# ViTAE-Transformer/MTP

Hardware: AMD Instinct MI355X
Metric: images/sec pretrain step (ViT-L+RVSA, 224^2, bf16) (higher is better)
Workload: dtype bf16; 1 GPU; ViT-L + RVSA backbone fwd+bwd + grad all-reduce + clip + AdamW, 224x224, batch 64 per GPU (BASELINE configs[2]/[3]); global_batch=64, parallelism=dp1, activation_checkpointing=False, heads=sum_i mean(f_i)

## Files before the change

### mtp_amd/csrc/elementwise.hip

```cpp
#include "common.h"

namespace {

template <typename T, bool INVERSE>
__global__ __launch_bounds__(256) void patchify_kernel(float* __restrict__ img, T* __restrict__ cols, int B, int Cin, int H, int W, int P, int Hp, int Wp) {
    const int K4 = Cin * P * P / 4, P4 = P / 4;
    const int64_t total = (int64_t)B * Hp * Wp * K4;
    for (int64_t i = (int64_t)blockIdx.x * 256 + threadIdx.x; i < total; i += (int64_t)gridDim.x * 256) {
        const int k4 = (int)(i % K4);
        const int64_t t = i / K4;
        const int kx4 = k4 % P4, ky = (k4 / P4) % P, c = k4 / (P4 * P);
        const int px = (int)(t % Wp), py = (int)((t / Wp) % Hp), b = (int)(t / ((int64_t)Wp * Hp));
        float* ip = img + (((int64_t)b * Cin + c) * H + py * P + ky) * W + px * P + kx4 * 4;
        T* cp = cols + t * (K4 * 4) + k4 * 4;
        if (INVERSE)
            *reinterpret_cast<float4*>(ip) = load4(cp);
        else
            store4(cp, *reinterpret_cast<const float4*>(ip));
    }
}

template <typename Ts, typename Td>
__global__ __launch_bounds__(256) void cast_kernel(const Ts* __restrict__ s, Td* __restrict__ d, int64_t n) {
    const int64_t n4 = n >> 2;
// ... 46 lines not shown
                }
            }
        }
    } else {
        const int64_t c = c0 + a;
        if (c < C) {
            const Tin* rp = ib + c * S + s0 + g;
#pragma unroll
            for (int v = 0; v < 4; ++v) {
                const int64_t s2 = s0 + g + 4 * v;
                if (s2 + 3 < S && (S & 3) == 0) {
                    const float4 x = load4(rp + 4 * v);
                    tile[a][g + 4 * v] = x.x; tile[a][g + 4 * v + 1] = x.y; tile[a][g + 4 * v + 2] = x.z; tile[a][g + 4 * v + 3] = x.w;
                } else {
                    for (int e = 0; e < 4; ++e)
                        if (s2 + e < S) tile[a][g + 4 * v + e] = Elem<Tin>::load(rp + 4 * v + e);
                }
            }
        }
        __syncthreads();
        const int64_t s = s0 + a;
        if (s < S) {
            Tout* wp = ob + pixel_to_row(s, Wp, L) * C + c0 + g;
#pragma unroll
            for (int v = 0; v < 4; ++v)
                if (c0 + g + 4 * v < C)
                    store4(wp + 4 * v, make_float4(tile[g + 4 * v][a], tile[g + 4 * v + 1][a], tile[g + 4 * v + 2][a], tile[g + 4 * v + 3][a]));
        }
    }
}

template <bool ROWS2COLS>
__global__ __launch_bounds__(256) void transpose8_bf16_kernel(const bf16_t* __restrict__ in, bf16_t* __restrict__ out, int64_t S, int64_t C, int Wp, int L) {
    __shared__ float tile[64][65];
    const int64_t bt = blockIdx.z;
    const int64_t s0 = (int64_t)blockIdx.x * 64, c0 = (int64_t)blockIdx.y * 64;
    const bf16_t* ib = in + bt * S * C;
    bf16_t* ob = out + bt * S * C;
    const int t = threadIdx.x, ra = t >> 3, cg = (t & 7) * 8;
    float x[8];
    if (ROWS2COLS) {
#pragma unroll
        for (int h = 0; h < 2; ++h) {
            const int64_t sp = s0 + ra + 32 * h;
            if (sp < S && c0 + cg < C) {
                load8(ib + pixel_to_row(sp, Wp, L) * C + c0 + cg, x);
#pragma unroll
                for (int e = 0; e < 8; ++e) tile[cg + e][ra + 32 * h] = x[e];
            }
        }
        __syncthreads();
#pragma unroll
        for (int h = 0; h < 2; ++h) {
            const int64_t c = c0 + ra + 32 * h;
            if (c < C && s0 + cg < S) {
#pragma unroll
                for (int e = 0; e < 8; ++e) x[e] = tile[ra + 32 * h][cg + e];
                store8(ob + c * S + s0 + cg, x);
            }
        }
    } else {
#pragma unroll
        for (int h = 0; h < 2; ++h) {
            const int64_t c = c0 + ra + 32 * h;
            if (c < C && s0 + cg < S) {
                load8(ib + c * S + s0 + cg, x);
#pragma unroll
                for (int e = 0; e < 8; ++e) tile[ra + 32 * h][cg + e] = x[e];
            }
        }
        __syncthreads();
#pragma unroll
        for (int h = 0; h < 2; ++h) {
            const int64_t sp = s0 + ra + 32 * h;
            if (sp < S && c0 + cg < C) {
#pragma unroll
                for (int e = 0; e < 8; ++e) x[e] = tile[cg + e][ra + 32 * h];
                store8(ob + pixel_to_row(sp, Wp, L) * C + c0 + cg, x);
            }
        }
    }
}

template <bool ROWS2COLS>
int launch_transpose(const void* in, int in_dt, void* out, int out_dt, int64_t batches, int64_t S, int64_t C, int Wp, int L, hipStream_t s) {
    if (C % 4) return MTP_ERR_ARG;
    dim3 grid((unsigned)((S + 63) / 64), (unsigned)((C + 63) / 64), (unsigned)batches), block(256);
    if (in_dt == MTP_BF16 && out_dt == MTP_BF16 && !(S & 7) && !(C & 7) && !(((uintptr_t)in | (uintptr_t)out) & 15)) {
        transpose8_bf16_kernel<ROWS2COLS><<<grid, block, 0, s>>>((const bf16_t*)in, (bf16_t*)out, S, C, Wp, L);
        return mtp_launch_status();
    }
    MTP_DISPATCH2(in_dt, out_dt, transpose_kernel<TA, TB, ROWS2COLS><<<grid, block, 0, s>>>((const TA*)in, (TB*)out, S, C, Wp, L));
    return mtp_launch_status();
}

template <typename T>
__global__ __launch_bounds__(256) void convt_pack_kernel(const float* __restrict__ w, T* __restrict__ wg, T* __restrict__ wgT, int64_t Cin, int64_t Cout) {
    const int64_t total = Cin * Cout * 4;
    for (int64_t i = (int64_t)blockIdx.x * 256 + threadIdx.x; i < total; i += (int64_t)gridDim.x * 256) {
        const int q = (int)(i & 3);
        const int64_t co = (i >> 2) % Cout, ci = (i >> 2) / Cout;
        const float v = w[i];
        if (wg) Elem<T>::store(wg + (q * Cout + co) * Cin + ci, v);
        if (wgT) Elem<T>::store(wgT + ci * (4 * Cout) + q * Cout + co, v);
    }
}
__global__ __launch_bounds__(256) void convt_unpack_kernel(const float* __restrict__ dwg, float* __restrict__ dw, int64_t Cin, int64_t Cout) {
    const int64_t total = Cin * Cout * 4;
    for (int64_t i = (int64_t)blockIdx.x * 256 + threadIdx.x; i < total; i += (int64_t)gridDim.x * 256) {
        const int q = (int)(i & 3);
        const int64_t co = (i >> 2) % Cout, ci = (i >> 2) / Cout;
        dw[i] = dwg[(q * Cout + co) * Cin + ci];
    }
}

template <typename T>
__global__ __launch_bounds__(256) void convt_pack_tiled_kernel(const float* __restrict__ w, T* __restrict__ wg, T* __restrict__ wgT, int Cin, int Cout) {
    __shared__ float tile[2][64][65];
    const int ci0 = blockIdx.y * 64, co0 = blockIdx.x * 64;
    const int t = threadIdx.x, lane = t & 63, wave = t >> 6, ra = t >> 3, cg = (t & 7) * 8;
    float4 v[16];
#pragma unroll
    for (int k = 0; k < 16; ++k) {
        const int ci = ci0 + wave + 4 * k, co = co0 + lane;
        v[k] = (ci < Cin && co < Cout) ? load4(w + ((int64_t)ci * Cout + co) * 4) : make_float4(0.f, 0.f, 0.f, 0.f);
    }
#pragma unroll
    for (int half = 0; half < 2; ++half) {
        if (half) __syncthreads();
#pragma unroll
        for (int k = 0; k < 16; ++k) {
            tile[0][wave + 4 * k][lane] = half ? v[k].z : v[k].x;
            tile[1][wave + 4 * k][lane] = half ? v[k].w : v[k].y;
        }
        __syncthreads();
        float o[8];
        if (wgT) {
            for (int l = ra; l < 128; l += 32) {
                const int r = l >> 1, qq = l & 1, ci = ci0 + r;
                if (ci < Cin && co0 + cg < Cout) {
#pragma unroll
                    for (int e = 0; e < 8; ++e) o[e] = tile[qq][r][cg + e];
                    store8(wgT + (int64_t)ci * 4 * Cout + (int64_t)(2 * half + qq) * Cout + co0 + cg, o);
                }
            }
        }
        if (wg) {
            for (int l = ra; l < 128; l += 32) {
                const int qq = l >> 6, c = l & 63, co = co0 + c;
                if (co < Cout && ci0 + cg < Cin) {
#pragma unroll
                    for (int e = 0; e < 8; ++e) o[e] = tile[qq][cg + e][c];
                    store8(wg + ((int64_t)(2 * half + qq) * Cout + co) * Cin + ci0 + cg, o);
                }
            }
        }
    }
}
__global__ __launch_bounds__(256) void convt_unpack_tiled_kernel(const float* __restrict__ dwg, float* __restrict__ dw, int Cin, int Cout) {
    __shared__ float tile[2][64][65];
    const int ci0 = blockIdx.y * 64, co0 = blockIdx.x * 64;
    const int t = threadIdx.x, lane = t & 63, wave = t >> 6, rb = t >> 4, c4 = (t & 15) * 4;
    float g[16][4];
#pragma unroll
    for (int half = 0; half < 2; ++half) {
        if (half) __syncthreads();
        for (int l = rb; l < 128; l += 16) {
            const int qq = l >> 6, c = l & 63, co = co0 + c;
            if (co < Cout && ci0 + c4 < Cin) {
                const float4 x = load4(dwg + ((int64_t)(2 * half + qq) * Cout + co) * Cin + ci0 + c4);
                tile[qq][c4 + 0][c] = x.x; tile[qq][c4 + 1][c] = x.y; tile[qq][c4 + 2][c] = x.z; tile[qq][c4 + 3][c] = x.w;
            }
        }
        __syncthreads();
// ... 280 lines not shown
```

### mtp_amd/engine.py

```python
import os

import torch

from . import ops
from .engine_base import EngineBase

F32 = torch.float32


class _Blk:
    __slots__ = ("window", "pre", "wqkv", "wqkvT", "wproj", "wprojT", "w1", "w1T", "w2", "w2T", "wsamp", "bsamp", "bproj", "b2", "wproj_s", "w2_s")


class BackboneEngine(EngineBase):
    def __init__(self, module, act_dtype=torch.bfloat16):
        super().__init__(module, act_dtype)
        self.C = module.embed_dim
        self.depth = len(module.blocks)
        self.heads = module.num_heads
        self.hd = self.C // self.heads
        self.scale = module.qk_scale if module.qk_scale is not None else self.hd ** -0.5
        self.window = [bool(w) for w in module.window_blocks]
        self.out_indices = list(module.out_indices)
        self._blk = None
        self._fpn = None
        self._pe = None
        self._ls = []
        self._zero_rel = {}

    def _fold_sources(self, P):
        with torch.no_grad():
            for pre, b in self._ls:
                g1, g2 = P[pre + "gamma_1"].detach(), P[pre + "gamma_2"].detach()
                torch.mul(P[pre + "attn.proj.weight"].detach(), g1[:, None], out=b.wproj_s)
                torch.mul(P[pre + "mlp.fc2.weight"].detach(), g2[:, None], out=b.w2_s)
                torch.mul(P[pre + "attn.proj.bias"].detach(), g1, out=b.bproj)
                torch.mul(P[pre + "mlp.fc2.bias"].detach(), g2, out=b.b2)

    def _pack_weights(self, P):
        for name, (wg, wgT) in self._fpn.items():
            ops.convt_pack(P[name + ".weight"].detach().contiguous(), wg, wgT)

    def fusable_images(self):
        return None if self._ls else self._wimg

    def _build_weight_images(self, P):
        dev = P["patch_embed.proj.weight"].device
        act, H, C = self.act, self.heads, self.C
        entries = []

        def both(w2d):
            w2d = w2d.detach()
            assert w2d.is_contiguous()
            R, Cc = w2d.shape
            wt = torch.empty(Cc, R, device=dev, dtype=act)
            w = w2d if act == F32 else torch.empty(R, Cc, device=dev, dtype=act)
            entries.append((w2d, None if act == F32 else w, wt, False))
            return w, wt

        ls = getattr(self.m, "init_values", None) is not None
        self._ls = []

        blks = []
        for i in range(self.depth):
            b = _Blk()
            b.window = self.window[i]
            b.pre = pre = "blocks.%d." % i
            b.wqkv, b.wqkvT = both(P[pre + "attn.qkv.weight"])
            b.bproj, b.b2 = P[pre + "attn.proj.bias"].detach(), P[pre + "mlp.fc2.bias"].detach()
            if ls:
                b.wproj_s, b.w2_s = torch.empty_like(P[pre + "attn.proj.weight"]), torch.empty_like(P[pre + "mlp.fc2.weight"])
                b.bproj, b.b2 = torch.empty_like(P[pre + "attn.proj.bias"]), torch.empty_like(P[pre + "mlp.fc2.bias"])
                self._ls.append((pre, b))
                b.wproj, b.wprojT = both(b.wproj_s)
            else:
                b.wproj, b.wprojT = both(P[pre + "attn.proj.weight"])
            b.w1, b.w1T = both(P[pre + "mlp.fc1.weight"])
            b.w2, b.w2T = both(b.w2_s if ls else P[pre + "mlp.fc2.weight"])
            if b.window:
                b.wsamp = torch.empty(5 * H, C, device=dev, dtype=F32)
                b.bsamp = torch.empty(5 * H, device=dev, dtype=F32)
                r0 = 0
                for head, rows in (("sampling_offsets", 2 * H), ("sampling_scales", 2 * H), ("sampling_angles", H)):
                    entries.append((P[pre + "attn.%s.2.weight" % head].detach().view(rows, C), b.wsamp[r0:r0 + rows], None, True))
                    entries.append((P[pre + "attn.%s.2.bias" % head].detach().view(1, rows), b.bsamp[r0:r0 + rows], None, True))
                    r0 += rows
            blks.append(b)
        self._blk = blks
        wpe = P["patch_embed.proj.weight"].detach()
        self._pe = both(wpe.view(wpe.shape[0], -1))
        fpn = {}
        for name in ("fpn1.0", "fpn1.3", "fpn2.0"):
            if name + ".weight" in P:
                Cin, Cout = P[name + ".weight"].shape[:2]
                fpn[name] = (torch.empty(4 * Cout, Cin, device=dev, dtype=act), torch.empty(Cin, 4 * Cout, device=dev, dtype=act))
        self._fpn = fpn
        self._wimg = ops.WeightImages(entries, act)

    wgrad_side_stream = True
    wgrad_max_jobs = 8
    wgrad_keep = 2

    @staticmethod
    def _colsum(dy, out):
        return ops.colsum(dy, out, accumulate=True)

    def _ln_bwd(self, *args, **kw):
        return ops.layernorm_bwd(*args, accumulate=True, defer=self._ln_parts, **kw)

    def _full_rel(self, pre, Hp, Wp):
        h = self.P.get(pre + "attn.full_attn_rel_pos_h")
        if h is not None:
            w = self.P[pre + "attn.full_attn_rel_pos_w"]
            if h.shape[0] < 2 * Hp - 1 or w.shape[0] < 2 * Wp - 1:
                raise ValueError("%sattn.full_attn_rel_pos_h/w have %d / %d rows, a %d x %d token grid needs %d / %d (resize them like "
                                 "init_weights does, or build the model for this input size)" % (pre, h.shape[0], w.shape[0], Hp, Wp, 2 * Hp - 1, 2 * Wp - 1))
            return h[:2 * Hp - 1], w[:2 * Wp - 1]
        key = (Hp, Wp)
        if self._zero_rel.get(key) is None:
            self._zero_rel[key] = (torch.zeros(2 * Hp - 1, self.hd, device=self.dev, dtype=F32),
                                   torch.zeros(2 * Wp - 1, self.hd, device=self.dev, dtype=F32))
        return self._zero_rel[key]

    def _drop_scales(self, B, training):
        rates = [float(self.m.drop_path_rates[i]) for i in range(self.depth)]
        live = [training and r > 0.0 and self.m.blocks[i].training for i, r in enumerate(rates)]
        if not any(live):
            return [(None, None)] * self.depth
        keep = torch.tensor([1.0 - r for r in rates], dtype=F32).to(self.dev, non_blocking=True).view(self.depth, 1, 1)
        s = torch.floor(keep + torch.rand(self.depth, 2, B, device=self.dev, dtype=F32)) / keep
        return [(s[i, 0], s[i, 1]) if live[i] else (None, None) for i in range(self.depth)]

    @property
    def _ride(self):
        return self.act == torch.bfloat16 and not self.m.use_checkpoint

    def _block_fwd(self, i, x, B, Hp, Wp, dps, save):
        P, b, C, T, N = self.P, self._blk[i], self.C, x.shape[0], Hp * Wp
        pre = b.pre
        s = {}
        mean1, rstd1 = self._e(T, dtype=F32), self._e(T, dtype=F32)
        ln1 = ops.layernorm_fwd(x, P[pre + "norm1.weight"], P[pre + "norm1.bias"], self._e(T, C), mean1, rstd1)
        rider = None
        if b.window:
            nh, nw = ops.rvsa_windows(Hp, Wp)
            R = B * nh * nw
            avg, pooled = self._e(R, C, dtype=F32), self._e(R, C, dtype=F32)
            samp = self._e(R, 5 * self.heads, dtype=F32)
            if self._ride:
                rider = ops.sampling_fwd_rider(ln1, b.wsamp, b.bsamp, avg, pooled, samp, B, Hp, Wp)
            else:
                ops.rvsa_sampling_fwd(ln1, b.wsamp, b.bsamp, avg, pooled, samp, B, Hp, Wp)
        qkv = ops.gemm_nt(ln1, b.wqkv, self._e(T, 3 * C), bias=P[pre + "attn.qkv.bias"], rider=rider)
        o = self._e(T, C)
        if b.window:
            lse = self._e(R * self.heads * 49, dtype=F32)
            ops.rvsa_attn_fwd(qkv, samp, o, lse, P[pre + "attn.rel_pos_h"], P[pre + "attn.rel_pos_w"],
                              P[pre + "attn.relative_position_bias_table"], B, Hp, Wp, self.heads, self.scale)
            s.update(avg=avg, pooled=pooled, samp=samp)
        else:
            lse = self._e(B * self.heads * N, dtype=F32)
            rel_h, rel_w = self._full_rel(pre, Hp, Wp)
            ops.full_attn_fwd(qkv, o, lse, rel_h, rel_w, B, Hp, Wp, self.heads, self.scale)
        x1 = ops.gemm_nt(o, b.wproj, self._e(T, C, dtype=F32), epi=ops.EPI_BIAS_RES, bias=b.bproj, res=x,
                         rowscale=dps[0], rows_per_sample=N)
        mean2, rstd2 = self._e(T, dtype=F32), self._e(T, dtype=F32)
        ln2 = ops.layernorm_fwd(x1, P[pre + "norm2.weight"], P[pre + "norm2.bias"], self._e(T, C), mean2, rstd2)
        u = self._e(T, 4 * C)
        h = ops.gemm_nt(ln2, b.w1, self._e(T, 4 * C), epi=ops.EPI_BIAS_GELU_DG, bias=P[pre + "mlp.fc1.bias"], aux=u)
        x2 = ops.gemm_nt(h, b.w2, self._e(T, C, dtype=F32), epi=ops.EPI_BIAS_RES, bias=b.b2, res=x1,
                         rowscale=dps[1], rows_per_sample=N)
        if save:
            s.update(x=x, mean1=mean1, rstd1=rstd1, ln1=ln1, qkv=qkv, o=o, lse=lse, x1=x1, mean2=mean2, rstd2=rstd2, ln2=ln2, u=u, h=h)
        return x2, s

    def _layer_scale_grads(self, pre, lin, gname, G):
        P = self.P
        gw, gb, gam = G[pre + lin + ".weight"], G[pre + lin + ".bias"], P[pre + gname]
        G[pre + gname].add_((gw * P[pre + lin + ".weight"]).sum(1) + gb * P[pre + lin + ".bias"])
        gw.mul_(gam[:, None])
        gb.mul_(gam)

    def _block_bwd(self, i, s, dx2, dx2_act, B, Hp, Wp, dps, G, extra, prev_scale):
        P, b, C, N = self.P, self._blk[i], self.C, Hp * Wp
        pre = b.pre
        T = dx2.shape[0]
        wq = self._wq
        ls = pre + "gamma_1" in G
# ... 66 lines not shown
        else:
            B, Cin, H, W = img.shape
            Hp, Wp = H // ps, W // ps
            N, T = Hp * Wp, B * Hp * Wp
            img = img.contiguous()
            if img.dtype != F32:
                img = img.float()
            cols = ops.patchify(img, self._e(T, Cin * ps * ps), ps)
        pos = P.get("pos_embed")
        if pos is not None:
            assert pos.shape[1] == N, "pos_embed does not match the input size"
            x = ops.gemm_nt(cols, self._pe[0], self._e(T, C, dtype=F32), epi=ops.EPI_BIAS_RES, bias=P["patch_embed.proj.bias"],
                            res=pos.reshape(N, C), res_mod=N)
        else:
            x = ops.gemm_nt(cols, self._pe[0], self._e(T, C, dtype=F32), bias=P["patch_embed.proj.bias"])
        dps = self._drop_scales(B, training)
        ckpt = bool(m.use_checkpoint) and need_grad
        saved, taps = [], {}
        vitdet = bool(getattr(m, "_vitdet", False))
        last = self.depth - 1 if vitdet else max(self.out_indices)
        for i in range(self.depth):
            if i > last:
                break
            xin = x
            x, s = self._block_fwd(i, x, B, Hp, Wp, dps[i], save=need_grad and not ckpt)
            saved.append(s if (need_grad and not ckpt) else ({"x": xin} if need_grad else None))
            if i in self.out_indices:
                taps[i] = x
        final = None
        if vitdet:
            fm, fr = self._e(T, dtype=F32), self._e(T, dtype=F32)
            xn = ops.layernorm_fwd(x, P["norm.weight"], P["norm.bias"], self._e(T, C, dtype=F32), fm, fr)
            final = (x, fm, fr)
            tap_list = [xn, xn, xn, xn]
        else:
            tap_list = [taps[i] for i in self.out_indices]
        if getattr(m, "_taps_only", False):
            feats = [ops.tokens_to_nchw(t, self._e(B, C, Hp, Wp, dtype=fdt), B, Hp, Wp, 0) for t in tap_list]
            fctx = {"taps_only": True}
        else:
            feats, fctx = self._fpn_fwd(tap_list, B, Hp, Wp, fdt, need_grad)
        ctx = None
        if need_grad:
            ctx = dict(saved=saved, dps=dps, fctx=fctx, cols=cols, geom=(B, Cin, H, W, Hp, Wp), ckpt=ckpt, last=last, final=final)
        return feats, ctx

    def _fpn_fwd(self, taps, B, Hp, Wp, fdt, need_grad):
        P, C, T = self.P, self.C, B * Hp * Wp
        m = self.m
        feats, fctx = [], {}
        if m.patch_size == 8:
            t0 = taps[0] if self.act == F32 else ops.cast(taps[0], self._e(T, C))
            z = ops.gemm_nt(t0, self._fpn["fpn1.0"][0], self._e(T, 4 * C), bias=P["fpn1.0.bias"], bias_mod=C)
            feats.append(ops.tokens_to_nchw(z.view(4 * T, C), self._e(B, C, 2 * Hp, 2 * Wp, dtype=fdt), B, Hp, Wp, 1))
            feats.append(ops.tokens_to_nchw(taps[1], self._e(B, C, Hp, Wp, dtype=fdt), B, Hp, Wp, 0))
            H2, W2, H4, W4 = Hp // 2, Wp // 2, Hp // 4, Wp // 4
            p3 = ops.maxpool2_tokens_fwd(taps[2], self._e(B * H2 * W2, C), B, Hp, Wp)
            feats.append(ops.tokens_to_nchw(p3, self._e(B, C, H2, W2, dtype=fdt), B, H2, W2, 0))
            q1 = ops.maxpool2_tokens_fwd(taps[3], self._e(B * H2 * W2, C, dtype=F32), B, Hp, Wp)
            q2 = ops.maxpool2_tokens_fwd(q1, self._e(B * H4 * W4, C), B, H2, W2)
            feats.append(ops.tokens_to_nchw(q2, self._e(B, C, H4, W4, dtype=fdt), B, H4, W4, 0))
            if need_grad:
                fctx = dict(p8=True, t0=t0, tap2=taps[2], tap3=taps[3], q1=q1)
            return feats, fctx
        if m.patch_size != 16:
            raise NotImplementedError("the reference defines the FPN tail for patch_size 16 and 8 only (VIT:640-670)")
        t0 = taps[0] if self.act == F32 else ops.cast(taps[0], self._e(T, C))
        y1 = ops.gemm_nt(t0, self._fpn["fpn1.0"][0], self._e(T, 4 * C), bias=P["fpn1.0.bias"], bias_mod=C)
        mean, rstd = self._e(4 * T, dtype=F32), self._e(4 * T, dtype=F32)
        g1 = ops.layernorm_fwd(y1.view(4 * T, C), P["fpn1.1.ln.weight"], P["fpn1.1.ln.bias"], self._e(4 * T, C), mean, rstd, gelu=True)
        y2 = ops.gemm_nt(g1, self._fpn["fpn1.3"][0], self._e(4 * T, 4 * C), bias=P["fpn1.3.bias"], bias_mod=C)
        feats.append(ops.tokens_to_nchw(y2.view(16 * T, C), self._e(B, C, 4 * Hp, 4 * Wp, dtype=fdt), B, Hp, Wp, 2))
        t1 = taps[1] if self.act == F32 else ops.cast(taps[1], self._e(T, C))
        z = ops.gemm_nt(t1, self._fpn["fpn2.0"][0], self._e(T, 4 * C), bias=P["fpn2.0.bias"], bias_mod=C)
        feats.append(ops.tokens_to_nchw(z.view(4 * T, C), self._e(B, C, 2 * Hp, 2 * Wp, dtype=fdt), B, Hp, Wp, 1))
        feats.append(ops.tokens_to_nchw(taps[2], self._e(B, C, Hp, Wp, dtype=fdt), B, Hp, Wp, 0))
        Ho, Wo = Hp // 2, Wp // 2
        pooled = ops.maxpool2_tokens_fwd(taps[3], self._e(B * Ho * Wo, C), B, Hp, Wp)
        feats.append(ops.tokens_to_nchw(pooled, self._e(B, C, Ho, Wo, dtype=fdt), B, Ho, Wo, 0))
        if need_grad:
            fctx = dict(t0=t0, y1=y1, mean=mean, rstd=rstd, g1=g1, t1=t1, tap3=taps[3])
        return feats, fctx

    def _convt_wgrad(self, dy, x, gw):
        dwg = self._e(dy.shape[1], x.shape[1], dtype=F32)
        self._wq.add(dy, x, dwg, after=lambda: ops.convt_unpack_grad(dwg, gw), norm_of=gw)

    def _fpn_bwd(self, dfeats, fctx, B, Hp, Wp, G):
        P, C, T, act = self.P, self.C, B * Hp * Wp, self.act
        out = [None] * 4

        def as_in(df):
            df = df.contiguous()
            return df if df.dtype in (F32, torch.bfloat16) else df.float()

        if fctx.get("p8"):
            H2, W2, H4, W4 = Hp // 2, Wp // 2, Hp // 4, Wp // 4
            if dfeats[0] is not None:
                dz = ops.nchw_to_tokens(as_in(dfeats[0]), self._e(4 * T, C), B, Hp, Wp, 1)
                self._convt_wgrad(dz.view(T, 4 * C), fctx["t0"], G["fpn1.0.weight"])
                self._colsum(dz, G["fpn1.0.bias"])
                out[0] = ops.gemm_nt(dz.view(T, 4 * C), self._fpn["fpn1.0"][1], self._e(T, C, dtype=F32))
            if dfeats[1] is not None:
                out[1] = ops.nchw_to_tokens(as_in(dfeats[1]), self._e(T, C, dtype=F32), B, Hp, Wp, 0)
            if dfeats[2] is not None:
                dp = ops.nchw_to_tokens(as_in(dfeats[2]), self._e(B * H2 * W2, C, dtype=F32), B, H2, W2, 0)
                out[2] = ops.maxpool2_tokens_bwd(fctx["tap2"], dp, self._e(T, C, dtype=F32), B, Hp, Wp)
            if dfeats[3] is not None:
                dq2 = ops.nchw_to_tokens(as_in(dfeats[3]), self._e(B * H4 * W4, C, dtype=F32), B, H4, W4, 0)
                dq1 = ops.maxpool2_tokens_bwd(fctx["q1"], dq2, self._e(B * H2 * W2, C, dtype=F32), B, H2, W2)
                out[3] = ops.maxpool2_tokens_bwd(fctx["tap3"], dq1, self._e(T, C, dtype=F32), B, Hp, Wp)
            return out

        if dfeats[0] is not None:
            dy2 = ops.nchw_to_tokens(as_in(dfeats[0]), self._e(16 * T, C), B, Hp, Wp, 2)
            self._convt_wgrad(dy2.view(4 * T, 4 * C), fctx["g1"], G["fpn1.3.weight"])
            self._colsum(dy2, G["fpn1.3.bias"])
            dg1 = ops.gemm_nt(dy2.view(4 * T, 4 * C), self._fpn["fpn1.3"][1], self._e(4 * T, C))
            dy1 = self._e(4 * T, C)
            self._ln_bwd(dg1, fctx["y1"].view(4 * T, C), fctx["mean"], fctx["rstd"], P["fpn1.1.ln.weight"], dy1,
                              G["fpn1.1.ln.weight"], G["fpn1.1.ln.bias"], beta=P["fpn1.1.ln.bias"], gelu=True)
            self._convt_wgrad(dy1.view(T, 4 * C), fctx["t0"], G["fpn1.0.weight"])
            self._colsum(dy1, G["fpn1.0.bias"])
            out[0] = ops.gemm_nt(dy1.view(T, 4 * C), self._fpn["fpn1.0"][1], self._e(T, C, dtype=F32))
        if dfeats[1] is not None:
            dz = ops.nchw_to_tokens(as_in(dfeats[1]), self._e(4 * T, C), B, Hp, Wp, 1)
            self._convt_wgrad(dz.view(T, 4 * C), fctx["t1"], G["fpn2.0.weight"])
            self._colsum(dz, G["fpn2.0.bias"])
            out[1] = ops.gemm_nt(dz.view(T, 4 * C), self._fpn["fpn2.0"][1], self._e(T, C, dtype=F32))
        if dfeats[2] is not None:
            out[2] = ops.nchw_to_tokens(as_in(dfeats[2]), self._e(T, C, dtype=F32), B, Hp, Wp, 0)
        if dfeats[3] is not None:
            Ho, Wo = Hp // 2, Wp // 2
            dp = ops.nchw_to_tokens(as_in(dfeats[3]), self._e(B * Ho * Wo, C, dtype=F32), B, Ho, Wo, 0)
            out[3] = ops.maxpool2_tokens_bwd(fctx["tap3"], dp, self._e(T, C, dtype=F32), B, Hp, Wp)
        return out

    def backward(self, ctx, dfeats, G, need_input_grad=False, on_block_done=None, split_last=False, sqn=None):
        B, Cin, H, W, Hp, Wp = ctx["geom"]
        C, N, T = self.C, Hp * Wp, B * Hp * Wp
        P = self.P
        self.dev = ctx["cols"].device
        wq = self._begin_backward(sqn)
        if ctx["fctx"].get("taps_only"):
            dtaps = [None if d is None else ops.nchw_to_tokens((d.contiguous() if d.dtype in (F32, torch.bfloat16) else d.float().contiguous()),
                                                               self._e(T, C, dtype=F32), B, Hp, Wp, 0) for d in dfeats]
        else:
            dtaps = self._fpn_bwd(dfeats, ctx["fctx"], B, Hp, Wp, G)
        tapgrad = {}
        last, dps, saved = ctx["last"], ctx["dps"], ctx["saved"]
        if ctx.get("final") is not None:
            dsum = None
            for d in dtaps:
                if d is None:
                    continue
                if dsum is None:
                    dsum = d
                else:
                    ops.axpy(dsum, d)
            if dsum is not None:
                xl, fm, fr = ctx["final"]
                tapgrad[last] = self._ln_bwd(dsum, xl, fm, fr, P["norm.weight"], self._e(T, C, dtype=F32), G["norm.weight"], G["norm.bias"])
        else:
            for idx, d in zip(self.out_indices, dtaps):
                if d is None:
                    continue
                if idx in tapgrad:
                    ops.axpy(tapgrad[idx], d)
                else:
                    tapgrad[idx] = d
        self._ln_flush()
        if on_block_done is not None and not wq.jobs:
            on_block_done(self.depth)
        if last not in tapgrad:
            tapgrad[last] = torch.zeros(T, C, device=self.dev, dtype=F32)
        dx = tapgrad[last]
        dx_act = self._scaled_copy(dx, dps[last][1], N)
        for i in range(last, -1, -1):
            s = saved[i]
            if ctx["ckpt"]:
                _, s = self._block_fwd(i, s["x"], B, Hp, Wp, dps[i], save=True)
            extra = tapgrad.get(i - 1) if i > 0 else None
            prev_scale = dps[i - 1][1] if i > 0 else None
            dx, dx_act = self._block_bwd(i, s, dx, dx_act, B, Hp, Wp, dps[i], G, extra, prev_scale)
            saved[i] = None
            if i == 0:
                wq.add(dx_act, ctx["cols"], G["patch_embed.proj.weight"].view(C, -1), G["patch_embed.proj.bias"])
            if i == 0 or wq.should_flush() or not wq.jobs or (split_last and i == 1):
                self._burst_out(i, on_block_done)
        self._wait_bursts()
        self._report_pending(on_block_done)
        if "pos_embed" in G:
            ops.reduce_rows(dx.view(B, N * C), G["pos_embed"])
        dimg = None
        if need_input_grad:
            dcols = ops.gemm_nt(dx_act, self._pe[1], self._e(T, ctx["cols"].shape[1]))
            dimg = ops.unpatchify(dcols, self._e(B, Cin, H, W, dtype=F32), self.m.patch_size)
        if on_block_done is not None:
            on_block_done(-1)
        return dimg

    def _scaled_copy(self, dx, scale, N):
        return ops.scale_rows_cast(dx, self._e(*dx.shape), scale, N)
```

### mtp_amd/ops.py

```python
import ctypes as C

import torch

from . import _lib
from ._lib import (EPI_BIAS, EPI_BIAS_GELU, EPI_BIAS_GELU_DG, EPI_BIAS_RES, EPI_DGELU, EPI_MUL, MTP_BF16, MTP_F32, GemmArgs,
                   check)
from ._lib import (GEMM_NT_FAMILY_P8, GEMM_NT_FAMILY_REG, GEMM_NT_FAMILY_SB, GEMM_NT_FAMILY_SB8, GEMM_NT_FAMILY_STRIP, GEMM_NT_NO_P8,
                   GEMM_NT_NO_PERSIST, GEMM_NT_NO_SB8, GEMM_NT_NO_STRIP, GEMM_NT_P8, GEMM_NT_P8_224, GEMM_NT_P8_256, GEMM_NT_PERSIST,
                   GEMM_NT_REG_STAGED, GEMM_NT_SB8, GEMM_NT_STRIP, GEMM_ORDER_GROUPED, GEMM_ORDER_PLAIN, GEMM_ORDER_ROW_MAJOR, GEMM_STORE_NT,
                   GEMM_STORE_PLAIN, GEMM_STORE_SC1, GEMM_TN_REG_TRANSPOSE, GEMM_TN_TR_FULL_ONLY, GEMM_TNG_PLAIN_ORDER, GEMM_TNG_PLAIN_PHASES)

_DT = {torch.float32: MTP_F32, torch.bfloat16: MTP_BF16}
def lib():
    return _lib.load()


def _dt(t):
    try:
        return _DT[t.dtype]
    except KeyError:
        raise TypeError("mtp_amd ops take float32 / bfloat16 tensors, got %s" % t.dtype)


def _p(t):
# ... 456 lines not shown
        keep.append((w, wt))
    return torch.frombuffer(bytearray(bytes(arr)), dtype=torch.uint8).to(device), tile0, keep


class WeightImages:

    def __init__(self, entries, act_dtype):
        rows = []
        for src, w, wt, f32_out in entries:
            assert src.dim() == 2 and src.dtype == torch.float32
            R, Cc = src.shape
            want = torch.float32 if f32_out else act_dtype
            for img in (w, wt):
                assert img is None or (img.dtype == want and img.numel() == R * Cc)
            rows.append((_f32(src), w, wt, R, Cc, f32_out, 0.0))
        self.table, self.total_tiles, self.keep = _wimg_table(rows, entries[0][0].device)
        self.n, self.act = len(rows), _DT[act_dtype]
        self.entries, self.act_dtype = list(entries), act_dtype

    def refresh(self):
        check(lib().mtp_weight_images(self.table.data_ptr(), self.n, self.total_tiles, self.act, _s()), "mtp_weight_images")


class AdamWImages:

    @staticmethod
    def build(flat, wimg, wd_of, lr_of=None):
        by_ptr = {}
        for src, w, wt, f32_out in (wimg.entries if wimg is not None else []):
            by_ptr[src.data_ptr()] = (src, w, wt, f32_out)
        base = flat.data.data_ptr()
        rows, scales = [], []
        used = 0
        for n in flat.names:
            if flat.groups[n] is None:
                continue
            off = flat.offsets[n]
            numel = 1
            for d in flat.shapes[n]:
                numel *= d
            ent = by_ptr.get(base + 4 * off)
            if ent is not None:
                src, w, wt, f32_out = ent
                if src.numel() != numel:
                    return None
                R, Cc = src.shape
                used += 1
            else:
                w = wt = None
                f32_out = False
                padded = (numel + 63) // 64 * 64
                R, Cc = padded // 64, 64
            rows.append((base + 4 * off, w, wt, R, Cc, f32_out, float(wd_of(n))))
            scales.append(1.0 if lr_of is None else float(lr_of(n)))
        if used != len(by_ptr):
            return None
        self = AdamWImages()
        self.table, self.total_tiles, self.keep = _wimg_table(rows, flat.data.device)
        self.n = len(rows)
        self.act = _DT[wimg.act_dtype] if wimg is not None else MTP_BF16
        self.lr = None if lr_of is None else torch.tensor(scales, dtype=torch.float32).to(flat.data.device)
        self.flat = flat
        return self

    def step(self, m, v, hyper, sqn, max_norm, grad_scale):
        f = self.flat
        fn, lr = ("mtp_adamw_weight_images", ()) if self.lr is None else ("mtp_adamw_weight_images_lr", (_f32(self.lr),))
        check(getattr(lib(), fn)(self.table.data_ptr(), *lr, self.n, self.total_tiles, self.act, _f32(f.data), _f32(f.grad), _f32(m), _f32(v), _f32(hyper),
                                 _f32(sqn), max_norm, grad_scale, _s()), fn)


def convt_pack(w, wg, wgT):
    Cin, Cout = w.shape[:2]
    dt = _dt(wg if wg is not None else wgT)
    check(lib().mtp_convt_pack(_f32(w), _p(wg), _p(wgT), dt, Cin, Cout, _s()), "mtp_convt_pack")


def convt_unpack_grad(dwg, dw):
    Cin, Cout = dw.shape[:2]
    check(lib().mtp_convt_unpack_grad(_f32(dwg), _f32(dw), Cin, Cout, _s()), "mtp_convt_unpack_grad")
    return dw


def tokens_to_nchw(x, out, B, Hp, Wp, levels):
    Cc = x.shape[-1]
    check(lib().mtp_tokens_to_nchw(_p(x), _dt(x), _p(out), _dt(out), B, Hp, Wp, Cc, levels, _s()), "mtp_tokens_to_nchw")
    return out


def nchw_to_tokens(f, out, B, Hp, Wp, levels):
    Cc = f.shape[1]
    check(lib().mtp_nchw_to_tokens(_p(f), _dt(f), _p(out), _dt(out), B, Hp, Wp, Cc, levels, _s()), "mtp_nchw_to_tokens")
    return out


def maxpool2_tokens_fwd(x, y, B, Hp, Wp):
    check(lib().mtp_maxpool2_tokens_fwd(_f32(x), _p(y), _dt(y), B, Hp, Wp, x.shape[-1], _s()), "mtp_maxpool2_tokens_fwd")
    return y


def maxpool2_tokens_bwd(x, dy, dx, B, Hp, Wp, accumulate=False):
    check(lib().mtp_maxpool2_tokens_bwd(_f32(x), _p(dy), _dt(dy), _f32(dx), int(accumulate), B, Hp, Wp, x.shape[-1], _s()), "mtp_maxpool2_tokens_bwd")
    return dx


def axpy(y, x, alpha=1.0):
    check(lib().mtp_axpy_f32(_f32(y), _f32(x), alpha, y.numel(), _s()), "mtp_axpy_f32")
    return y


def scale_rows_cast(src, dst, scale=None, rows_per_sample=0):
    rows, Cc = src.shape
    check(lib().mtp_scale_rows_cast(_f32(src), _p(dst), _dt(dst), _f32(scale), rows_per_sample, rows, Cc, _s()), "mtp_scale_rows_cast")
    return dst


def full_attn_fwd(qkv, o, lse, rel_h, rel_w, B, Hp, Wp, heads, scale):
    hd = qkv.shape[1] // (3 * heads)
    check(lib().mtp_full_attn_fwd(_p(qkv), _p(o), _f32(lse), _dt(qkv), _f32(rel_h), _f32(rel_w), B, Hp, Wp, heads, hd, scale, _s()), "mtp_full_attn_fwd")
    return o, lse


def full_attn_bwd(qkv, o, dout, lse, dqkv, rel_h, rel_w, drel_h, drel_w, B, Hp, Wp, heads, scale, accumulate=False, defer=None):
    hd = qkv.shape[1] // (3 * heads)
    rt = (2 * Hp - 1) + (2 * Wp - 1)
    part = _scratch((B * heads, rt * hd), qkv.device, torch.float32)
    nws = lib().mtp_full_attn_bwd_workspace_floats(B, Hp, Wp, heads)
    ws = _scratch((nws,), qkv.device, torch.float32) if nws else None
    check(lib().mtp_full_attn_bwd(_p(qkv), _p(o), _p(dout), _f32(lse), _p(dqkv), _dt(qkv), _f32(rel_h), _f32(rel_w), _p(part), _p(ws),
                                  B, Hp, Wp, heads, hd, scale, _s()), "mtp_full_attn_bwd")
    if defer is not None and _adjacent(drel_h, drel_w) and drel_h.numel() == (2 * Hp - 1) * hd:
        defer.append((part, drel_h, accumulate))
        return dqkv
    _reduce_pair(part, (2 * Hp - 1) * hd, drel_h, drel_w, accumulate)
    return dqkv


FULL_FWD = {"v3": 1, "flash128": 3, "flash256": 4, "generic": 5}
FULL_BWD = {"v3": 1, "flash": 3, "three_pass": 4, "single_wg": 5}
RVSA_FWD = {"generic": 1, "mfma": 2}
RVSA_BWD = {"generic": 1, "mfma_dense": 2, "mfma_atomic": 3}


def full_attn_kernel(dtype, Hp, Wp, backward=False):
    rc = lib().mtp_full_attn_kernel(_DT[dtype], Hp, Wp, int(backward))
    if rc < 0:
        check(rc, "mtp_full_attn_kernel")
    return rc


def rvsa_attn_kernel(dtype, Hp, Wp, heads, backward=False):
    rc = lib().mtp_rvsa_attn_kernel(_DT[dtype], Hp, Wp, heads, int(backward))
    if rc < 0:
        check(rc, "mtp_rvsa_attn_kernel")
    return rc


def rvsa_windows(Hp, Wp):
    nh = (Hp + (7 - Hp % 7) % 7) // 7
    nw = (Wp + (7 - Wp % 7) % 7) // 7
    return nh, nw


def rvsa_pool_fwd(x, avg, pooled, B, Hp, Wp):
    check(lib().mtp_rvsa_pool_fwd(_p(x), _dt(x), _f32(avg), _f32(pooled), B, Hp, Wp, x.shape[-1], _s()), "mtp_rvsa_pool_fwd")

# ... 946 lines not shown
```

Baseline: 1906 images/sec.

## Fuse FPN convT bias colsum into wgrad queue and add persistent f32↔bf16 transpose

Two changes. In the FPN backward, the transposed-conv bias gradient is no longer a separate colsum pass over dy; it is folded into the deferred weight-gradient GEMM job through a colsum buffer, then reduced and zeroed after the job finishes. Separately, a new persistent 128x128-tile transpose kernel pair handles f32 rows to bf16 channel-major layout and back, with swizzled LDS and software prefetch of the next tile. This replaces the generic 64x64 transpose for those mixed-dtype cases and adds a per-name cached buffer and more complex kernels.

```diff
diff --git a/mtp_amd/csrc/elementwise.hip b/mtp_amd/csrc/elementwise.hip
--- a/mtp_amd/csrc/elementwise.hip
+++ b/mtp_amd/csrc/elementwise.hip
@@ -152,14 +152,176 @@
     }
 }
 
+constexpr int kTrS = 128, kTrC = 128;
+constexpr int kTrRowUnits = (kTrS / 2) * (kTrC / 8) / 256;
+constexpr int kTrColUnits = kTrC * (kTrS / 8) / 256;
+constexpr int kTrGrid = 1024;
+
+__device__ __forceinline__ int tr_word(int c, int p) { return c * (kTrS / 2) + (p ^ (((c >> 3) & 7) << 2)); }
+
+__device__ __forceinline__ uint32_t tr_spread_bits(uint32_t v) {
+    v = (v | (v << 8)) & 0x00ff00ffu; v = (v | (v << 4)) & 0x0f0f0f0fu; v = (v | (v << 2)) & 0x33333333u;
+    return (v | (v << 1)) & 0x55555555u;
+}
+__device__ __forceinline__ int64_t pixel_to_row32(uint32_t s, uint32_t Wp, int L) {
+    const uint32_t Wo = Wp << L, y = s / Wo, x = s - y * Wo, m = (1u << L) - 1u;
+    return ((((y >> L) * Wp + (x >> L)) << (2 * L)) | (tr_spread_bits(y & m) << 1) | tr_spread_bits(x & m));
+}
+
+typedef __attribute__((ext_vector_type(4))) uint32_t tr_u4_t;
+struct TrRows {
+    f32x4_t lo0, lo1, hi0, hi1;
+    __device__ __forceinline__ void load(const float* a, const float* b) {
+        lo0 = *reinterpret_cast<const f32x4_t*>(a); lo1 = *reinterpret_cast<const f32x4_t*>(a + 4);
+        hi0 = *reinterpret_cast<const f32x4_t*>(b); hi1 = *reinterpret_cast<const f32x4_t*>(b + 4);
+    }
+    __device__ __forceinline__ void store(float* a, float* b) const {
+        *reinterpret_cast<f32x4_t*>(a) = lo0; *reinterpret_cast<f32x4_t*>(a + 4) = lo1;
+        *reinterpret_cast<f32x4_t*>(b) = hi0; *reinterpret_cast<f32x4_t*>(b + 4) = hi1;
+    }
+    __device__ __forceinline__ void words(uint32_t (&w)[8]) const {
+#pragma unroll
+        for (int i = 0; i < 4; ++i) {
+            w[i] = pack_bf16x2(lo0[i], hi0[i]);
+            w[4 + i] = pack_bf16x2(lo1[i], hi1[i]);
+        }
+    }
+    __device__ __forceinline__ void from_words(const uint32_t (&w)[8]) {
+#pragma unroll
+        for (int i = 0; i < 4; ++i) {
+            lo0[i] = bf16_bits_to_f32(w[i] & 0xffffu); hi0[i] = bf16_bits_to_f32(w[i] >> 16);
+            lo1[i] = bf16_bits_to_f32(w[4 + i] & 0xffffu); hi1[i] = bf16_bits_to_f32(w[4 + i] >> 16);
+        }
+    }
+};
+
+struct TrTile {
+    int64_t base;
+    int s0, c0;
+};
+__device__ __forceinline__ TrTile tr_locate(int t, int S, int C, int tiles_s, int tiles_c) {
+    const int r = t / tiles_s, bt = r / tiles_c;
+    return {(int64_t)bt * S * C, (t - r * tiles_s) * kTrS, (r - bt * tiles_c) * kTrC};
+}
+
+__device__ __forceinline__ bool tr_row_unit(const TrTile& w, int k, int tid, int S, int C, int Wp, int L, int64_t& off) {
+    const int s = w.s0 + 2 * ((tid >> 4) + 16 * k), c = w.c0 + 8 * (tid & 15);
+    const bool ok = s < S && c < C;
+    off = w.base + pixel_to_row32(ok ? s : 0, Wp, L) * C + (ok ? c : 0);
+    return ok;
+}
+__device__ __forceinline__ bool tr_col_unit(const TrTile& w, int k, int tid, int S, int C, int64_t& off) {
+    const int c = w.c0 + (tid >> 4) + 16 * k, s = w.s0 + 8 * (tid & 15);
+    const bool ok = s < S && c < C;
+    off = w.base + (int64_t)(ok ? c : 0) * S + (ok ? s : 0);
+    return ok;
+}
+
+__global__ __launch_bounds__(256) void tokens_to_cs_stream_kernel(const float* __restrict__ rows, bf16_t* __restrict__ cols, int S, int C, int Wp, int L, int tiles_s,
+                                                                 int tiles_c, int ntiles) {
+    __shared__ __attribute__((aligned(16))) uint32_t tile[kTrC * kTrS / 2];
+    const int tid = threadIdx.x, rcg = tid & 15, rp0 = tid >> 4, cj = tid & 15, cc0 = tid >> 4;
+    TrRows r[kTrRowUnits];
+    int64_t off;
+    int t = blockIdx.x;
+    if (t >= ntiles) return;
+    TrTile w = tr_locate(t, S, C, tiles_s, tiles_c);
+#pragma unroll
+    for (int k = 0; k < kTrRowUnits; ++k) {
+        tr_row_unit(w, k, tid, S, C, Wp, L, off);
+        r[k].load(rows + off, rows + off + C);
+    }
+    for (;;) {
+#pragma unroll
+        for (int k = 0; k < kTrRowUnits; ++k) {
+            uint32_t x[8];
+            r[k].words(x);
+#pragma unroll
+            for (int e = 0; e < 8; ++e) tile[tr_word(8 * rcg + e, rp0 + 16 * k)] = x[e];
+        }
+        __syncthreads();
+        const int tn = t + (int)gridDim.x;
+        const bool more = tn < ntiles;
+        const TrTile wn = tr_locate(more ? tn : t, S, C, tiles_s, tiles_c);
+#pragma unroll
+        for (int k = 0; k < kTrRowUnits; ++k) {
+            tr_row_unit(wn, k, tid, S, C, Wp, L, off);
+            r[k].load(rows + off, rows + off + C);
+        }
+#pragma unroll
+        for (int k = 0; k < kTrColUnits; ++k) {
+            const tr_u4_t v = *reinterpret_cast<const tr_u4_t*>(&tile[tr_word(cc0 + 16 * k, 4 * cj)]);
+            if (tr_col_unit(w, k, tid, S, C, off)) *reinterpret_cast<tr_u4_t*>(cols + off) = v;
+        }
+        if (!more) return;
+        __syncthreads();
+        t = tn;
+        w = wn;
+    }
+}
+
+__global__ __launch_bounds__(256) void cs_to_tokens_stream_kernel(const bf16_t* __restrict__ cols, float* __restrict__ rows, int S, int C, int Wp, int L, int tiles_s,
+                                                                 int tiles_c, int ntiles) {
+    __shared__ __attribute__((aligned(16))) uint32_t tile[kTrC * kTrS / 2];
+    const int tid = threadIdx.x, rcg = tid & 15, rp0 = tid >> 4, cj = tid & 15, cc0 = tid >> 4;
+    tr_u4_t q[kTrColUnits];
+    int64_t off;
+    int t = blockIdx.x;
+    if (t >= ntiles) return;
+    TrTile w = tr_locate(t, S, C, tiles_s, tiles_c);
+#pragma unroll
+    for (int k = 0; k < kTrColUnits; ++k) {
+        tr_col_unit(w, k, tid, S, C, off);
+        q[k] = *reinterpret_cast<const tr_u4_t*>(cols + off);
+    }
+    for (;;) {
+#pragma unroll
+        for (int k = 0; k < kTrColUnits; ++k) *reinterpret_cast<tr_u4_t*>(&tile[tr_word(cc0 + 16 * k, 4 * cj)]) = q[k];
+        __syncthreads();
+        const int tn = t + (int)gridDim.x;
+        const bool more = tn < ntiles;
+        const TrTile wn = tr_locate(more ? tn : t, S, C, tiles_s, tiles_c);
+#pragma unroll
+        for (int k = 0; k < kTrColUnits; ++k) {
+            tr_col_unit(wn, k, tid, S, C, off);
+            q[k] = *reinterpret_cast<const tr_u4_t*>(cols + off);
+        }
+#pragma unroll
+        for (int k = 0; k < kTrRowUnits; ++k) {
+            uint32_t x[8];
+#pragma unroll
+            for (int e = 0; e < 8; ++e) x[e] = tile[tr_word(8 * rcg + e, rp0 + 16 * k)];
+            TrRows v;
+            v.from_words(x);
+            if (tr_row_unit(w, k, tid, S, C, Wp, L, off)) v.store(rows + off, rows + off + C);
+        }
+        if (!more) return;
+        __syncthreads();
+        t = tn;
+        w = wn;
+    }
+}
+
 template <bool ROWS2COLS>
 int launch_transpose(const void* in, int in_dt, void* out, int out_dt, int64_t batches, int64_t S, int64_t C, int Wp, int L, hipStream_t s) {
     if (C % 4) return MTP_ERR_ARG;
-    dim3 grid((unsigned)((S + 63) / 64), (unsigned)((C + 63) / 64), (unsigned)batches), block(256);
-    if (in_dt == MTP_BF16 && out_dt == MTP_BF16 && !(S & 7) && !(C & 7) && !(((uintptr_t)in | (uintptr_t)out) & 15)) {
+    const bool vec8 = !(S & 7) && !(C & 7) && !(((uintptr_t)in | (uintptr_t)out) & 15);
+    if (vec8 && in_dt == MTP_BF16 && out_dt == MTP_BF16) {
+        dim3 grid((unsigned)((S + 63) / 64), (unsigned)((C + 63) / 64), (unsigned)batches), block(256);
         transpose8_bf16_kernel<ROWS2COLS><<<grid, block, 0, s>>>((const bf16_t*)in, (bf16_t*)out, S, C, Wp, L);
         return mtp_launch_status();
     }
+    const int64_t tiles_s = (S + kTrS - 1) / kTrS, tiles_c = (C + kTrC - 1) / kTrC, ntiles = tiles_s * tiles_c * batches;
+    if (vec8 && (ROWS2COLS ? in_dt : out_dt) == MTP_F32 && (ROWS2COLS ? out_dt : in_dt) == MTP_BF16 && S < (1ll << 31) - kTrS && C < (1ll << 31) - kTrC &&
+        ntiles > 0 && ntiles < (1 << 30) && L <= 15) {
+        const unsigned grid = (unsigned)(ntiles < kTrGrid ? ntiles : kTrGrid);
+        if (ROWS2COLS)
+            tokens_to_cs_stream_kernel<<<grid, 256, 0, s>>>((const float*)in, (bf16_t*)out, (int)S, (int)C, Wp, L, (int)tiles_s, (int)tiles_c, (int)ntiles);
+        else
+            cs_to_tokens_stream_kernel<<<grid, 256, 0, s>>>((const bf16_t*)in, (float*)out, (int)S, (int)C, Wp, L, (int)tiles_s, (int)tiles_c, (int)ntiles);
+        return mtp_launch_status();
+    }
+    dim3 grid((unsigned)((S + 63) / 64), (unsigned)((C + 63) / 64), (unsigned)batches), block(256);
     MTP_DISPATCH2(in_dt, out_dt, transpose_kernel<TA, TB, ROWS2COLS><<<grid, block, 0, s>>>((const TA*)in, (TB*)out, S, C, Wp, L));
     return mtp_launch_status();
 }
diff --git a/mtp_amd/engine.py b/mtp_amd/engine.py
--- a/mtp_amd/engine.py
+++ b/mtp_amd/engine.py
@@ -27,6 +27,7 @@
         self._pe = None
         self._ls = []
         self._zero_rel = {}
+        self._convt_cs = {}
 
     def _fold_sources(self, P):
         with torch.no_grad():
@@ -100,10 +101,6 @@
     wgrad_side_stream = True
     wgrad_max_jobs = 8
     wgrad_keep = 2
-
-    @staticmethod
-    def _colsum(dy, out):
-        return ops.colsum(dy, out, accumulate=True)
 
     def _ln_bwd(self, *args, **kw):
         return ops.layernorm_bwd(*args, accumulate=True, defer=self._ln_parts, **kw)
@@ -336,9 +333,11 @@
             fctx = dict(t0=t0, y1=y1, mean=mean, rstd=rstd, g1=g1, t1=t1, tap3=taps[3])
         return feats, fctx
 
-    def _convt_wgrad(self, dy, x, gw):
-        dwg = self._e(dy.shape[1], x.shape[1], dtype=F32)
-        self._wq.add(dy, x, dwg, after=lambda: ops.convt_unpack_grad(dwg, gw), norm_of=gw)
+    def _convt_wgrad(self, dy, x, name, G):
+        cs = self._convt_cs.get(name)
+        if cs is None or cs.device != dy.device or cs.numel() != dy.shape[1]:
+            cs = self._convt_cs[name] = torch.zeros(dy.shape[1], device=dy.device, dtype=F32)
+        ops.convt_wgrad(self._wq, dy, x, self._e(dy.shape[1], x.shape[1], dtype=F32), G[name + ".weight"], G[name + ".bias"], cs)
 
     def _fpn_bwd(self, dfeats, fctx, B, Hp, Wp, G):
         P, C, T, act = self.P, self.C, B * Hp * Wp, self.act
@@ -352,8 +351,7 @@
             H2, W2, H4, W4 = Hp // 2, Wp // 2, Hp // 4, Wp // 4
             if dfeats[0] is not None:
                 dz = ops.nchw_to_tokens(as_in(dfeats[0]), self._e(4 * T, C), B, Hp, Wp, 1)
-                self._convt_wgrad(dz.view(T, 4 * C), fctx["t0"], G["fpn1.0.weight"])
-                self._colsum(dz, G["fpn1.0.bias"])
+                self._convt_wgrad(dz.view(T, 4 * C), fctx["t0"], "fpn1.0", G)
                 out[0] = ops.gemm_nt(dz.view(T, 4 * C), self._fpn["fpn1.0"][1], self._e(T, C, dtype=F32))
             if dfeats[1] is not None:
                 out[1] = ops.nchw_to_tokens(as_in(dfeats[1]), self._e(T, C, dtype=F32), B, Hp, Wp, 0)
@@ -368,19 +366,16 @@
 
         if dfeats[0] is not None:
             dy2 = ops.nchw_to_tokens(as_in(dfeats[0]), self._e(16 * T, C), B, Hp, Wp, 2)
-            self._convt_wgrad(dy2.view(4 * T, 4 * C), fctx["g1"], G["fpn1.3.weight"])
-            self._colsum(dy2, G["fpn1.3.bias"])
+            self._convt_wgrad(dy2.view(4 * T, 4 * C), fctx["g1"], "fpn1.3", G)
             dg1 = ops.gemm_nt(dy2.view(4 * T, 4 * C), self._fpn["fpn1.3"][1], self._e(4 * T, C))
             dy1 = self._e(4 * T, C)
             self._ln_bwd(dg1, fctx["y1"].view(4 * T, C), fctx["mean"], fctx["rstd"], P["fpn1.1.ln.weight"], dy1,
                               G["fpn1.1.ln.weight"], G["fpn1.1.ln.bias"], beta=P["fpn1.1.ln.bias"], gelu=True)
-            self._convt_wgrad(dy1.view(T, 4 * C), fctx["t0"], G["fpn1.0.weight"])
-            self._colsum(dy1, G["fpn1.0.bias"])
+            self._convt_wgrad(dy1.view(T, 4 * C), fctx["t0"], "fpn1.0", G)
             out[0] = ops.gemm_nt(dy1.view(T, 4 * C), self._fpn["fpn1.0"][1], self._e(T, C, dtype=F32))
         if dfeats[1] is not None:
             dz = ops.nchw_to_tokens(as_in(dfeats[1]), self._e(4 * T, C), B, Hp, Wp, 1)
-            self._convt_wgrad(dz.view(T, 4 * C), fctx["t1"], G["fpn2.0.weight"])
-            self._colsum(dz, G["fpn2.0.bias"])
+            self._convt_wgrad(dz.view(T, 4 * C), fctx["t1"], "fpn2.0", G)
             out[1] = ops.gemm_nt(dz.view(T, 4 * C), self._fpn["fpn2.0"][1], self._e(T, C, dtype=F32))
         if dfeats[2] is not None:
             out[2] = ops.nchw_to_tokens(as_in(dfeats[2]), self._e(T, C, dtype=F32), B, Hp, Wp, 0)
diff --git a/mtp_amd/ops.py b/mtp_amd/ops.py
--- a/mtp_amd/ops.py
+++ b/mtp_amd/ops.py
@@ -562,6 +562,17 @@
     return dw
 
 
+def convt_wgrad(wq, dy, x, dwg, dw, db, cs):
+    assert cs.dtype == torch.float32 and cs.numel() == dy.shape[1] == 4 * db.numel() and cs.is_contiguous()
+
+    def after():
+        convt_unpack_grad(dwg, dw)
+        reduce_rows(cs.view(4, -1), db, accumulate=True)
+        cs.zero_()
+
+    return wq.add(dy, x, dwg, colsum=cs, after=after, norm_of=dw)
+
+
 def tokens_to_nchw(x, out, B, Hp, Wp, levels):
     Cc = x.shape[-1]
     check(lib().mtp_tokens_to_nchw(_p(x), _dt(x), _p(out), _dt(out), B, Hp, Wp, Cc, levels, _s()), "mtp_tokens_to_nchw")
```

Result: no change. 1914 images/sec, median of 6 (+0.4%).
